# maxnorman569/Variational-Gridded-Gaussian-Processes

Measured on AMD Instinct MI355X. Metric: ELBO-step grid-points/sec (value + 5-component gradient), 1024x1024 RBF grid per GPU, higher is better.
Workload: dtype f64; 1 GPU; 2D Kronecker rbf GP (points basis), 1024x1024 grid (1024x1024 per GPU), m_d=128, Adam fit loop (lr 0.01), eigensolver warm start on; parallelism=single GPU

## Files before the change

include/vggp.h:

```cpp
#ifndef VGGP_H
#define VGGP_H

#include <stdint.h>

#ifdef __cplusplus
extern "C" {
#endif

#define VGGP_VERSION 200

#define VGGP_OK        0
#define VGGP_EINVAL   -1
#define VGGP_ENOTPD   -2
#define VGGP_EHIP     -3
#define VGGP_ENOMEM   -4
#define VGGP_ESTATE   -5
#define VGGP_ENOCONV  -6
#define VGGP_ERCCL    -7

#define VGGP_KIND_MATERN12 0
#define VGGP_KIND_MATERN32 1
#define VGGP_KIND_MATERN52 2
#define VGGP_KIND_RBF      3

// ... 131 lines not shown
                              double* var, vggp_info* info, void* stream);
int vggp_exact_readout_iter(vggp_ctx* ctx, const double* C1, int64_t mv1, const double* C2, int64_t mv2, const double* kd1,
                            const double* kd2, const int64_t* cells, int64_t n_cells, double tol, int max_iter, double* mean, double* var,
                            int flags, vggp_info* info, void* stream);

int vggp_exact_kmv(vggp_ctx* ctx, int kind1, int kind2, double ell1, double ell2, const double* xr1, const double* xr2, int64_t Nr,
                   const double* xc1, const double* xc2, int64_t Nc, const double* V, int64_t nb, double* out0, double* out1, double* out2,
                   void* stream);

int vggp_factor_build(vggp_ctx* ctx, int kind, int basis, const double* x, int64_t n,
                      const double* grid, int64_t m, double ell, int flags,
                      double* A0, double* dA0, double* K0, double* dK0, void* stream);

int vggp_cholesky_inverse(vggp_ctx* ctx, const double* K, int64_t m, double* L, double* Linv,
                          double* jitter_out, void* stream);

int vggp_eigh(vggp_ctx* ctx, const double* G, int64_t m, double* lam, double* Qt,
              int32_t* sweeps_out, int flags, void* stream);

int vggp_gemm(vggp_ctx* ctx, const double* A, int64_t sa_m, int64_t sa_k,
              const double* B, int64_t sb_k, int64_t sb_n,
              double* C, int64_t ldc, int64_t M, int64_t N, int64_t K, void* stream);

int vggp_trsm(vggp_ctx* ctx, const double* L, int64_t m, const double* R, int64_t ncols, double* X, int trans, void* stream);

int vggp_kron_solve(vggp_ctx* ctx, const double* L1, int64_t n1, const double* L2, int64_t n2,
                    const double* Y, double* X, void* stream);

#define VGGP_NSTAGE 20
int         vggp_profile(vggp_ctx* ctx, int enable);
int         vggp_profile_read(vggp_ctx* ctx, double ms_out[VGGP_NSTAGE], int32_t* steps_out, int reset);
const char* vggp_stage_name(int stage);
const char* vggp_project_kernel_name(void);

int vggp_sumsq(vggp_ctx* ctx, const double* y, int64_t n, double* out, void* stream);

#ifdef __cplusplus
}
#endif
#endif
```

variational_gridded_gaussian_processes_amd/_lib.py:

```python
from __future__ import annotations

import ctypes as C
import os

HERE = os.path.dirname(os.path.abspath(__file__))
LIB_PATH = os.path.join(HERE, "libvggp_hip.so")

VGGP_OK, VGGP_EINVAL, VGGP_ENOTPD, VGGP_EHIP, VGGP_ENOMEM, VGGP_ESTATE, VGGP_ENOCONV, VGGP_ERCCL = 0, -1, -2, -3, -4, -5, -6, -7
UNIQUE_ID_BYTES = 128
ALLREDUCE_FN = C.CFUNCTYPE(C.c_int, C.c_void_p, C.POINTER(C.c_double), C.c_int64)
KIND = {"matern12": 0, "matern32": 1, "matern52": 2, "rbf": 3}
NSTAGE = 20
FLAG_B0_F32_KDELTA = 1
FLAG_BLOCK_JACOBI = 2
FLAG_SCATTERED = 4
FLAG_PAIRED_Z = 8
BASIS = {"points": 0, "b0": 1, "one": 2, "vff": 3, "b1": 4}


class VggpError(RuntimeError):
    def __init__(self, code: int, msg: str):
        super().__init__(f"libvggp_hip: {msg} (code {code})")
        self.code = code


class Desc(C.Structure):
    _fields_ = [("kind1", C.c_int32), ("basis1", C.c_int32), ("kind2", C.c_int32), ("basis2", C.c_int32),
                ("n1", C.c_int64), ("n2", C.c_int64), ("m1", C.c_int64), ("m2", C.c_int64),
                ("n_total", C.c_int64),
                ("x1", C.c_void_p), ("x2", C.c_void_p), ("grid1", C.c_void_p), ("grid2", C.c_void_p),
                ("warm_start", C.c_int32), ("flags", C.c_int32)]


class Info(C.Structure):
    _fields_ = [("jitter1", C.c_double), ("jitter2", C.c_double),
                ("sweeps1", C.c_int32), ("sweeps2", C.c_int32),
                ("rounds1", C.c_int32), ("rounds2", C.c_int32),
                ("status", C.c_int32), ("polished", C.c_int32)]

# ... 39 lines not shown
    "vggp_zgrad_scattered": (_I, [_P, _P, _P, _P, _P]),
    "vggp_set_inducing": (_I, [_P, C.c_int, _P, C.c_int64]),
    "vggp_posterior": (_I, [_P, _P, _P, _I64, _P, _P, _P]),
    "vggp_readout": (_I, [_P, _P, _I64, _P, _I64, _P, _P, _P, _P, _I, _P]),
    "vggp_readout_masked": (_I, [_P, _P, _I64, _P, _I64, _P, _P, _P, _P, _I, _P]),
    "vggp_posterior_masked": (_I, [_P, _P, _P, _I64, _P, _P, _P]),
    "vggp_posterior_cov": (_I, [_P, _P, _P, _I64, _P, _P]),
    "vggp_posterior_cov_masked": (_I, [_P, _P, _P, _I64, _P, _P]),
    "vggp_qv_cov_masked": (_I, [_P, _P, _P]),
    "vggp_exact_plan": (_I, [_P, _I, _I, _P, _P, _I64]),
    "vggp_exact_step": (_I, [_P, _P, C.POINTER(_D), C.POINTER(_D), C.POINTER(_D), C.POINTER(Info), _P]),
    "vggp_exact_posterior": (_I, [_P, _P, _P, _I64, _P, _P, _P]),
    "vggp_exact_posterior_cov": (_I, [_P, _P, _P, _I64, _P, _P]),
    "vggp_exact_readout": (_I, [_P, _P, _I64, _P, _I64, _P, _P, _P, _P, _I, _P]),
    "vggp_exact_iter_plan": (_I, [_P, _I, _I, _P, _P, _I64]),
    "vggp_exact_step_iter": (_I, [_P, _P, C.POINTER(_D), _I, _I, _D, _I, C.POINTER(_D), C.POINTER(_D), C.POINTER(Info), _P]),
    "vggp_exact_posterior_iter": (_I, [_P, _P, _P, _I64, _D, _I, _P, _P, C.POINTER(Info), _P]),
    "vggp_exact_readout_iter": (_I, [_P, _P, _I64, _P, _I64, _P, _P, C.POINTER(_I64), _I64, _D, _I, _P, _P, _I, C.POINTER(Info), _P]),
    "vggp_exact_kmv": (_I, [_P, _I, _I, _D, _D, _P, _P, _I64, _P, _P, _I64, _P, _I64, _P, _P, _P, _P]),
    "vggp_factor_build": (_I, [_P, _I, _I, _P, _I64, _P, _I64, _D, _I, _P, _P, _P, _P, _P]),
    "vggp_cholesky_inverse": (_I, [_P, _P, _I64, _P, _P, C.POINTER(_D), _P]),
    "vggp_eigh": (_I, [_P, _P, _I64, _P, _P, C.POINTER(C.c_int32), _I, _P]),
    "vggp_gemm": (_I, [_P, _P, _I64, _I64, _P, _I64, _I64, _P, _I64, _I64, _I64, _I64, _P]),
    "vggp_kron_solve": (_I, [_P, _P, _I64, _P, _I64, _P, _P, _P]),
    "vggp_trsm": (_I, [_P, _P, _I64, _P, _I64, _P, _I, _P]),
    "vggp_sumsq": (_I, [_P, _P, _I64, C.POINTER(_D), _P]),
    "vggp_profile": (_I, [_P, _I]),
    "vggp_profile_read": (_I, [_P, C.POINTER(_D), C.POINTER(C.c_int32), _I]),
    "vggp_stage_name": (C.c_char_p, [_I]),
    "vggp_project_kernel_name": (C.c_char_p, []),
}

_lib = None


def load() -> C.CDLL:
    global _lib
    if _lib is not None:
        return _lib
    if not os.path.exists(LIB_PATH):
        raise ImportError(
            f"{LIB_PATH} not found: build it with `python -m variational_gridded_gaussian_processes_amd.build` "
            "(needs hipcc); there is no CPU fallback")
    lib = C.CDLL(LIB_PATH)
    for name, (res, args) in SYMBOLS.items():
        fn = getattr(lib, name)
# ... 11 lines not shown
```

variational_gridded_gaussian_processes_amd/csrc/api.hip:

```cpp
#include "common.h"

#include <math.h>
#include <stdarg.h>
#include <stdio.h>
#include <stdlib.h>
#include <string.h>
#include <time.h>

#include <algorithm>
#include <vector>

static thread_local char g_err[512] = "";
void vg_set_error(const char* fmt, ...) {
    va_list ap;
    va_start(ap, fmt);
    vsnprintf(g_err, sizeof(g_err), fmt, ap);
    va_end(ap);
}
extern "C" const char* vggp_last_error(void) { return g_err; }
extern "C" int vggp_version(void) { return VGGP_VERSION; }

#include "ctx.h"
#include "factor_elem.h"
#define VG_CHOL_MAXJOBS_HOST 8
// ... 2061 lines not shown
    j.err = counters + 4;
    VG_HIP(vg_eigh_launch(&j, 1, st));
    int hc[8] = {0, 0, 0, 0, 0, 0, 0, 0};
    VG_HIP(hipMemcpyAsync(hc, counters, sizeof(hc), hipMemcpyDeviceToHost, st));
    VG_HIP(hipStreamSynchronize(st));
    if (sweeps_out) *sweeps_out = hc[1] & 0xff;
    if (hc[2] || hc[4]) { vg_set_error("vggp_eigh: no convergence"); return VGGP_ENOCONV; }
    return VGGP_OK;
}

extern "C" int vggp_gemm(vggp_ctx* c, const double* A, int64_t sa_m, int64_t sa_k, const double* B, int64_t sb_k,
                         int64_t sb_n, double* C, int64_t ldc, int64_t M, int64_t N, int64_t K, void* stream) {
    if (!c) { vg_set_error("null context"); return VGGP_EINVAL; }
    VG_REQUIRE(A && B && C && M >= 1 && N >= 1 && K >= 1 && ldc >= N, "vggp_gemm: bad argument");
    VG_REQUIRE(M < (1L << 30) && N < (1L << 30) && K < (1L << 30), "vggp_gemm: dimension too large");
    VG_ENTER_DEVICE(c->device);
    VgGemmBatch g;
    vg_gemm_init(&g);
    vg_gemm_add(&g, A, sa_m, sa_k, B, sb_k, sb_n, C, (int)ldc, (int)M, (int)N, (int)K);
    VG_HIP(vg_gemm_launch(&g, stream ? (hipStream_t)stream : c->own_stream));
    return VGGP_OK;
}

extern "C" int vggp_trsm(vggp_ctx* c, const double* L, int64_t m, const double* R, int64_t ncols, double* X, int trans,
                         void* stream) {
    if (!c) { vg_set_error("null context"); return VGGP_EINVAL; }
    VG_REQUIRE(L && R && X && m >= 1 && m <= 16384 && ncols >= 1, "vggp_trsm: bad argument (1 <= m <= 16384)");
    VG_REQUIRE(m * ncols < (1L << 31) && m * m < (1L << 31), "vggp_trsm: matrix too large");
    VG_ENTER_DEVICE(c->device);
    hipStream_t st = stream ? (hipStream_t)stream : c->own_stream;
    const long nb16 = (m + 15) / 16;
    int rc = vg_ensure_misc(c, (size_t)nb16 * 256 * sizeof(double));
    if (rc) return rc;
    double* Dinv = (double*)c->misc;
    VG_HIP(vg_tri_diaginv_launch(L, m, (int)m, Dinv, st));
    if (X != R) VG_HIP(hipMemcpyAsync(X, R, sizeof(double) * m * ncols, hipMemcpyDeviceToDevice, st));
    return trsm_inplace(L, m, m, Dinv, X, ncols, 1, ncols, trans ? 1 : 0, st);
}

struct VgTriInvSpec { const double* L; long n; const double* Dinv16; double* Xinv; double* tmp; };
static int tri_inverse_batch(const VgTriInvSpec* sp, int nf, hipStream_t st) {
    VgTrsmJob tj[16];
    int nt = 0;
    for (int f = 0; f < nf; ++f)
        for (long r0 = 0; r0 < sp[f].n; r0 += VG_TRSM_BLK) {
            const long rb = std::min<long>(VG_TRSM_BLK, sp[f].n - r0);
// ... 278 lines not shown
```

variational_gridded_gaussian_processes_amd/csrc/common.h:

```cpp
#pragma once
#if defined(__HIP_DEVICE_COMPILE__) && !defined(__gfx950__)
#error "libvggp_hip is written for gfx950 (MI355X) only: kernels rely on its wave64 barrier semantics, MFMA shapes and LDS size"
#endif
#include <hip/hip_runtime.h>
#include <stdint.h>
#include "../../include/vggp.h"

#define VG_WAVE 64

void vg_set_error(const char* fmt, ...);
#define VG_HIP(call)                                                              \
    do {                                                                          \
        hipError_t _e = (call);                                                   \
        if (_e != hipSuccess) {                                                   \
            vg_set_error("%s:%d: %s -> %s", __FILE__, __LINE__, #call,            \
                         hipGetErrorString(_e));                                  \
            return VGGP_EHIP;                                                     \
        }                                                                         \
    } while (0)
#define VG_REQUIRE(cond, ...)                                                     \
    do {                                                                          \
        if (!(cond)) {                                                            \
            vg_set_error(__VA_ARGS__);                                            \
            return VGGP_EINVAL;                                                   \
// ... 42 lines not shown
    double* dot_out;
    int dotw_ld;
    int deep;
    int rev;
};
#define VG_TRI_NONE 0
#define VG_TRI_A_LOWER 1
#define VG_TRI_A_UPPER 2
#define VG_TRI_B_UPPER 3
#define VG_TRI_B_LOWER 4
#define VG_TRI_A_UPPER_B_LOWER 5
struct VgGemmBatch {
    int nprob;
    int total_tiles;
    VgGemmP p[VG_GEMM_MAXP];
};

void vg_gemm_init(VgGemmBatch* b);
int vg_gemm_add(VgGemmBatch* b, const double* A, long sa_m, long sa_k, const double* B, long sb_k,
                long sb_n, double* C, int ldc, int M, int N, int K, int ksplit = 1, long c_slab = 0,
                int b_nslab = 1, long b_slab = 0, double alpha = 1.0, int accum = 0);
#define VG_GEMM_TAG_GRAM_PROJECT 1
#define VG_GEMM_TAG_WIDE 2
void vg_gemm_xcd_group(VgGemmBatch* b, int prob);
hipError_t vg_gemm_launch(const VgGemmBatch* b, hipStream_t st, int tag = 0);
const char* vg_last_project_kernel();

#define VG_RED_MAXSEG 8
struct VgRedSeg { const double* in; double* out; long n; long slab; int nslab; int block_start; };
struct VgRedBatch { int nseg; int total_blocks; VgRedSeg s[VG_RED_MAXSEG]; };
void vg_red_init(VgRedBatch* b);
void vg_red_add(VgRedBatch* b, const double* in, double* out, long n, long slab, int nslab);
hipError_t vg_red_launch(const VgRedBatch* b, hipStream_t st);

struct VgFactorJob {
    const double* x;
    const double* grid;
    double* A0;
    double* dA0;
    double* K0;
    double* dK0;
    int n, m, kind, basis;
    int theta_idx;
    double ell_imm;
    int flags;
};
// ... 183 lines not shown
```

variational_gridded_gaussian_processes_amd/csrc/gemm.hip:

```cpp
#include "gemm_body.h"

#include <cstdint>
#include <cstdio>
#include <cstdlib>

__global__ __launch_bounds__(256) void vg_gemm_kernel(const VgGemmBatch b) {
    __shared__ double lds[2 * VgTile<64, 16>::TILE];
    vg_gemm_body<64, 16>(b, lds, blockIdx.x);
}
__global__ __launch_bounds__(256) void vg_gemm_gram_project_kernel(const VgGemmBatch b) {
    __shared__ double lds[2 * VgTile<64, 16>::TILE];
    vg_gemm_body<64, 16>(b, lds, blockIdx.x);
}
__global__ __launch_bounds__(512) void vg_gemm_gram_project_wide_kernel(const VgGemmBatch b) {
    __shared__ double lds[2 * VgTile<64, 16>::TILE];
    vg_gemm_body<64, 16, 512>(b, lds, blockIdx.x);
}
typedef double vg_d2 __attribute__((ext_vector_type(2)));
__global__ __launch_bounds__(512) void vg_gemm_project_deep_kernel(const VgGemmBatch b) {
    constexpr int T = 64, NT = 512, BK = 32;
    constexpr int RS = BK + 2;
    constexpr int KS = T + 16;
    constexpr int NA = T * BK / (2 * NT);
    __shared__ __attribute__((aligned(16))) double lds[T * RS + BK * KS];
// ... 184 lines not shown
        for (int i = 0; i < out->nprob; ++i) {
            const VgGemmP& p = out->p[i];
            fprintf(stderr, "[deep] NOT deep: prob %d/%d M %d N %d K %d ksplit %d kchunk %d sa (%ld,%ld) sb (%ld,%ld) aslab %d bslab %d tri %d accum %d tiles %d deep %d\n",
                    i, out->nprob, p.M, p.N, p.K, p.ksplit, p.kchunk, p.sa_m, p.sa_k, p.sb_k, p.sb_n, p.a_nslab, p.b_nslab, p.tri, p.accum,
                    p.tiles_m * p.tiles_n * p.ksplit, p.deep);
        }
    return 4 * deep_tiles >= 3L * out->total_tiles;
}
__global__ __launch_bounds__(512) void vg_gemm_deep_kernel(const VgGemmBatch b) {
    constexpr int DT = 32 * 80 > 64 * 34 ? 32 * 80 : 64 * 34;
    __shared__ __attribute__((aligned(16))) double lds[2 * DT];
    const int bid = blockIdx.x;
    int pi = 0;
    for (int i = 1; i < b.nprob; ++i)
        if (bid >= b.p[i].tile_start) pi = i;
    if (b.p[pi].deep) vg_gemm_deep_body(b.p[pi], lds, bid - b.p[pi].tile_start);
    else vg_gemm_body<64, 16, 512>(b, lds, bid);
}
__global__ __launch_bounds__(512) void vg_gemm_wide_kernel(const VgGemmBatch b) {
    __shared__ double lds[2 * VgTile<64, 16>::TILE];
    vg_gemm_body<64, 16, 512>(b, lds, blockIdx.x);
}
__global__ __launch_bounds__(256) void vg_gemm_small_kernel(const VgGemmBatch b) {
    __shared__ double lds[2 * VgTile<32, 32>::TILE];
    vg_gemm_body<32, 32>(b, lds, blockIdx.x);
}

void vg_gemm_init(VgGemmBatch* b) {
    b->nprob = 0;
    b->total_tiles = 0;
}

int vg_gemm_add(VgGemmBatch* b, const double* A, long sa_m, long sa_k, const double* B, long sb_k,
                long sb_n, double* C, int ldc, int M, int N, int K, int ksplit, long c_slab,
                int b_nslab, long b_slab, double alpha, int accum) {
    if (b->nprob >= VG_GEMM_MAXP) return -1;
    VgGemmP& p = b->p[b->nprob];
    p.A = A; p.B = B; p.C = C;
    p.sa_m = sa_m; p.sa_k = sa_k; p.sb_k = sb_k; p.sb_n = sb_n;
    p.M = M; p.N = N; p.K = K; p.ldc = ldc;
    p.alpha = alpha; p.accum = accum;
    if (ksplit < 1) ksplit = 1;
    int ktiles = (K + VG_BK - 1) / VG_BK;
    if (ktiles < 1) ktiles = 1;
    if (ksplit > ktiles) ksplit = ktiles;
    int per = (ktiles + ksplit - 1) / ksplit;
// ... 11 lines not shown
    p.dotw = nullptr; p.dot_out = nullptr; p.dotw_ld = 0; p.deep = 0;
    p.tiles_m = (M + VG_BM - 1) / VG_BM;
    p.tiles_n = (N + VG_BN - 1) / VG_BN;
    p.tile_start = b->total_tiles;
    b->total_tiles += p.tiles_m * p.tiles_n * ksplit;
    return b->nprob++;
}

void vg_gemm_xcd_group(VgGemmBatch* b, int prob) {
    static const bool off = getenv("VGGP_NO_XCD_GROUP") != nullptr;
    VgGemmP& p = b->p[prob];
    const bool ok = !off && p.tile_start == 0 && (p.ksplit == 1 || p.ksplit == 2 || p.ksplit == 4 || p.ksplit == 8) &&
                    (p.tiles_n % (8 / p.ksplit)) == 0;
    p.xcd_group = ok ? 1 : 0;
}

static bool vg_deep_batch(const VgGemmBatch* b, VgGemmBatch* out);

static const char* g_last_project_kernel = "";
const char* vg_last_project_kernel() { return g_last_project_kernel; }

hipError_t vg_gemm_launch(const VgGemmBatch* b, hipStream_t st, int tag) {
    if (b->nprob == 0 || b->total_tiles == 0) return hipSuccess;
    bool small = b->total_tiles < 128;
    for (int i = 0; i < b->nprob; ++i) small = small && b->p[i].ksplit == 1 && b->p[i].K <= 512;
    if (small) {
        VgGemmBatch s = *b;
        s.total_tiles = 0;
        for (int i = 0; i < s.nprob; ++i) {
            VgGemmP& p = s.p[i];
            p.tiles_m = (p.M + 31) / 32;
            p.tiles_n = (p.N + 31) / 32;
            p.kchunk = ((p.K + 31) / 32) * 32;
            p.xcd_group = 0;
            p.tile_start = s.total_tiles;
            s.total_tiles += p.tiles_m * p.tiles_n;
        }
        hipLaunchKernelGGL(vg_gemm_small_kernel, dim3(s.total_tiles), dim3(256), 0, st, s);
        return hipGetLastError();
    }
    static const bool wide = getenv("VGGP_GEMM_NARROW") == nullptr;
    VgGemmBatch deepb;
    if (tag == VG_GEMM_TAG_GRAM_PROJECT && wide && vg_project_deep_ok(b)) {
        g_last_project_kernel = "vg_gemm_project_deep_kernel";
        hipLaunchKernelGGL(vg_gemm_project_deep_kernel, dim3(b->total_tiles), dim3(512), 0, st, *b);
    } else if (tag == VG_GEMM_TAG_GRAM_PROJECT && wide && b->total_tiles <= 320) {
        g_last_project_kernel = "vg_gemm_gram_project_wide_kernel";
        hipLaunchKernelGGL(vg_gemm_gram_project_wide_kernel, dim3(b->total_tiles), dim3(512), 0, st, *b);
    } else if (tag == VG_GEMM_TAG_GRAM_PROJECT) {
        g_last_project_kernel = "vg_gemm_gram_project_kernel";
        hipLaunchKernelGGL(vg_gemm_gram_project_kernel, dim3(b->total_tiles), dim3(256), 0, st, *b);
    }
    else if (vg_deep_batch(b, &deepb)) {
        hipLaunchKernelGGL(vg_gemm_deep_kernel, dim3(deepb.total_tiles), dim3(512), 0, st, deepb);
    }
    else if (tag == VG_GEMM_TAG_WIDE && wide && b->total_tiles <= 320)
        hipLaunchKernelGGL(vg_gemm_wide_kernel, dim3(b->total_tiles), dim3(512), 0, st, *b);
    else
        hipLaunchKernelGGL(vg_gemm_kernel, dim3(b->total_tiles), dim3(256), 0, st, *b);
    return hipGetLastError();
}
// ... 38 lines not shown
```

variational_gridded_gaussian_processes_amd/csrc/gemm_body.h:

```cpp
#pragma once
#include "common.h"

typedef double vg_d4 __attribute__((ext_vector_type(4)));

template <int T, int BK>
struct VgTile {
    static constexpr int RPAD = BK == 16 ? 1 : 4;
    static constexpr int RS = BK + RPAD;
    static constexpr int KS = T + 16;
    static constexpr int TILE = (BK * KS > T * RS) ? BK * KS : T * RS;
    static constexpr int MB = T / 32;
};

template <int T, int BK, int NT = 256>
__device__ __forceinline__ void vg_gemm_body(const VgGemmBatch& b, double* lds, const int bid) {
    using C_ = VgTile<T, BK>;
    constexpr int NR = T * BK / NT;
    constexpr int WC = NT / 128;
    constexpr int MB = T / 32;
    constexpr int NB = T / (16 * WC);
    double* As = lds;
    double* Bs = lds + C_::TILE;

    int pi = 0;
    for (int i = 1; i < b.nprob; ++i)
        if (bid >= b.p[i].tile_start) pi = i;
    const VgGemmP& p = b.p[pi];

    int t = bid - p.tile_start;
    const int tiles = p.tiles_m * p.tiles_n;
    int ks, tm, tn;
    if (p.xcd_group) {
        const int nx = 8 / p.ksplit;
        const int xcd = t & 7, j = t >> 3;
        ks = xcd / nx;
        const int gi = j / p.tiles_m;
        tm = j - gi * p.tiles_m;
// ... 90 lines not shown
            Bs[b_k[r] * b_sk + b_j[r] * b_sj] = rb[r];
        }
        __syncthreads();
        if (knext < k_end) load_tile(knext, ra, rb);
#pragma unroll
        for (int kk = 0; kk < BK; kk += 4) {
            double av[MB], bv[NB];
#pragma unroll
            for (int mb = 0; mb < MB; ++mb)
                av[mb] = As[(wr * WT + mb * 16 + fi) * a_si + (kk + fk) * a_sk];
#pragma unroll
            for (int nb = 0; nb < NB; ++nb)
                bv[nb] = Bs[(kk + fk) * b_sk + (wc * WTC + nb * 16 + fi) * b_sj];
#pragma unroll
            for (int mb = 0; mb < MB; ++mb)
#pragma unroll
                for (int nb = 0; nb < NB; ++nb)
                    acc[mb][nb] = __builtin_amdgcn_mfma_f64_16x16x4f64(av[mb], bv[nb], acc[mb][nb], 0, 0, 0);
        }
        __syncthreads();
    };
    const bool fast = row0 + T <= M && col0 + T <= N && k_begin < k_end && ((k_end - k_begin) % BK) == 0 &&
                      ((nslab == 1 && anslab == 1) || p.K <= 512);
    if (fast) {
        const double* pa[NR];
        const double* pb[NR];
        int la[NR], lb[NR];
#pragma unroll
        for (int r = 0; r < NR; ++r) {
            pa[r] = A + (long)(row0 + a_i[r]) * sa_m + (long)(k_begin + a_k[r]) * sa_k;
            pb[r] = B + (long)(k_begin + b_k[r]) * sb_k + (long)(col0 + b_j[r]) * sb_n;
            la[r] = a_i[r] * a_si + a_k[r] * a_sk;
            lb[r] = b_k[r] * b_sk + b_j[r] * b_sj;
        }
        const long da = (long)BK * sa_k, db = (long)BK * sb_k;
        const int nk = (k_end - k_begin) / BK;
        auto ld = [&](double (&ra)[NR], double (&rb)[NR]) {
#pragma unroll
            for (int r = 0; r < NR; ++r) { ra[r] = *pa[r]; rb[r] = *pb[r]; }
            for (int sl = 1; sl < nslab; sl += 3) {
                const long o0 = (long)sl * bslab, o1 = sl + 1 < nslab ? o0 + bslab : o0, o2 = sl + 2 < nslab ? o0 + 2 * bslab : o0;
                const double w1 = sl + 1 < nslab ? 1.0 : 0.0, w2 = sl + 2 < nslab ? 1.0 : 0.0;
#pragma unroll
                for (int r = 0; r < NR; ++r) rb[r] += (pb[r][o0] + w1 * pb[r][o1]) + w2 * pb[r][o2];
            }
            for (int sl = 1; sl < anslab; sl += 3) {
                const long o0 = (long)sl * aslab, o1 = sl + 1 < anslab ? o0 + aslab : o0, o2 = sl + 2 < anslab ? o0 + 2 * aslab : o0;
// ... 77 lines not shown
```

variational_gridded_gaussian_processes_amd/csrc/thin.hip:

```cpp
#include "common.h"

typedef double vt_d4 __attribute__((ext_vector_type(4)));

#define VT_MAXR 32
#define VT_NBUF 15
#define VT_NBIG 11
#define VT_NSMALL 14
#ifdef VGGP_DIAG
#define VT_STAMP(i) do { if (threadIdx.x == 0 && tt.stamps) { unsigned long long t_; asm volatile("s_memrealtime %0\n\ts_waitcnt lgkmcnt(0)" : "=s"(t_) :: "memory"); tt.stamps[i] = t_; } } while (0)
#else
#define VT_STAMP(i)
#endif

struct VtTask { int c, a, sa_i, sa_k, b; };

__device__ __forceinline__ void vt_mm(double* base, int sz, const VtTask* tk, int ntask, int mp, int ld, int kk) {
    const int lane = threadIdx.x & 63, wave = threadIdx.x >> 6, nw = blockDim.x >> 6, nb = mp >> 4;
    const int fi = lane & 15, fk = lane >> 4;
    for (int t = wave; t < ntask * nb * nb; t += nw) {
        const int task = t / (nb * nb), blk = t - task * nb * nb, bi = blk / nb, bj = blk - bi * nb;
        const VtTask T = tk[task];
        const double* a = base + (long)T.a * sz + (bi * 16 + fi) * T.sa_i + fk * T.sa_k;
        const double* b = base + (long)T.b * sz + fk * ld + bj * 16 + fi;
        double* C = base + (long)T.c * sz;
// ... 27 lines not shown
        for (int q = 0; q < NV; ++q) t[q] = __shfl_xor(v[q], off);
#pragma unroll
        for (int q = 0; q < NV; ++q) v[q] += t[q];
    }
}

enum { B_W1 = 0, B_W1T, B_W2, B_W2T, B_E1, B_F1, B_E2, B_F2, B_P0, B_P1, B_P2, B_T0, B_T1, B_T2, B_T3 };

__global__ __launch_bounds__(1024) void vg_thin_tail_kernel(const VgThinTail tt) {
    extern __shared__ __attribute__((aligned(16))) double vt_dyn[];
    __shared__ double red[16 * VT_NBIG], tot[VT_NBIG + VT_NSMALL];
    __shared__ double dg[4][256];
    __shared__ double l1s[VT_MAXR], l2s[VT_MAXR], rs1[VT_MAXR], rl1[VT_MAXR], rs2[VT_MAXR], rl2[VT_MAXR];
    __shared__ VtTask tk[18];
    __shared__ double stage[16];
    __shared__ double jit_s[2], pf_s, seq_s;
    __shared__ int rc_s[2][4], st_s[2][2];
    const int r1 = tt.r1, r2 = tt.r2, tid = threadIdx.x, nthr = blockDim.x;
    const int rmax = r1 > r2 ? r1 : r2, mp = (rmax + 15) & ~15, ld = mp + 2, sz = mp * ld;
    double* base = vt_dyn;
    const double s1 = tt.theta[2], s2 = tt.theta[3], v = tt.theta[4];

    VT_STAMP(0);
    for (int e = tid; e < sz; e += nthr) {
        const int i = e / ld, j = e - i * ld;
        const bool in1 = i < r1 && j < r1, in2 = i < r2 && j < r2, in12 = i < r1 && j < r2;
        const double w1 = in1 ? tt.W1[i * r1 + j] : 0.0, w2 = in2 ? tt.W2[i * r2 + j] : 0.0;
        const double am1 = in1 ? tt.AM1[i * r1 + j] : 0.0, ah1 = in1 ? tt.AH1[i * r1 + j] : 0.0;
        const double am2 = in2 ? tt.AM2[i * r2 + j] : 0.0, ah2 = in2 ? tt.AH2[i * r2 + j] : 0.0;
        double c0 = 0.0, c1 = 0.0, c2 = 0.0;
        if (in12)
            for (int sl = 0; sl < tt.ac_nslab; ++sl) {
                const double* ac = tt.AC + sl * tt.ac_slab + i * r2 + j;
                c0 += ac[0]; c1 += ac[(long)r1 * r2]; c2 += ac[2L * r1 * r2];
            }
        base[B_W1 * sz + e] = w1; base[B_W2 * sz + e] = w2;
        if (j < mp) { base[B_W1T * sz + j * ld + i] = w1; base[B_W2T * sz + j * ld + i] = w2; }
        base[B_E1 * sz + e] = am1; base[B_F1 * sz + e] = ah1; base[B_E2 * sz + e] = am2; base[B_F2 * sz + e] = ah2;
        base[B_P0 * sz + e] = c0; base[B_P1 * sz + e] = c1; base[B_P2 * sz + e] = c2;
    }
    if (tid < VT_MAXR) {
        l1s[tid] = tid < r1 ? s1 * tt.lam1[tid] : 0.0;
        l2s[tid] = tid < r2 ? s2 * tt.lam2[tid] : 0.0;
    }
    if (tid >= 64 && tid < 72) { const int k = (tid - 64) >> 2, q = (tid - 64) & 3; rc_s[k][q] = tt.rcounters[k] ? tt.rcounters[k][q] : 0; }
    if (tid >= 72 && tid < 76) { const int k = (tid - 72) >> 1, q = (tid - 72) & 1; st_s[k][q] = tt.status[k] ? tt.status[k][q] : 0; }
    if (tid >= 76 && tid < 78) jit_s[tid - 76] = tt.jit[tid - 76] ? *tt.jit[tid - 76] : 0.0;
    if (tid == 78) pf_s = tt.peer_fail ? *tt.peer_fail : 0.0;
    if (tid == 79) seq_s = tt.theta[5];
    if (tid >= 128 && tid < 384) {
        const int i = tid - 128;
        dg[0][i] = i < tt.m1 ? tt.G1[(long)i * tt.m1 + i] : 0.0; dg[1][i] = i < tt.m1 ? tt.H1[(long)i * tt.m1 + i] : 0.0;
        dg[2][i] = i < tt.m2 ? tt.G2[(long)i * tt.m2 + i] : 0.0; dg[3][i] = i < tt.m2 ? tt.H2[(long)i * tt.m2 + i] : 0.0;
    }
    if (tid == 0) {
        tk[0] = VtTask{B_T0, B_E1, ld, 1, B_W1T}; tk[1] = VtTask{B_T1, B_F1, ld, 1, B_W1T};
        tk[2] = VtTask{B_T2, B_E2, ld, 1, B_W2T}; tk[3] = VtTask{B_T3, B_F2, ld, 1, B_W2T};
        tk[4] = VtTask{B_E1, B_W1, ld, 1, B_T0}; tk[5] = VtTask{B_F1, B_W1, ld, 1, B_T1};
        tk[6] = VtTask{B_E2, B_W2, ld, 1, B_T2}; tk[7] = VtTask{B_F2, B_W2, ld, 1, B_T3};
        tk[8] = VtTask{B_T0, B_P0, ld, 1, B_W2T}; tk[9] = VtTask{B_T1, B_P1, ld, 1, B_W2T}; tk[10] = VtTask{B_T2, B_P2, ld, 1, B_W2T};
        tk[11] = VtTask{B_P0, B_W1, ld, 1, B_T0}; tk[12] = VtTask{B_P1, B_W1, ld, 1, B_T1}; tk[13] = VtTask{B_P2, B_W1, ld, 1, B_T2};
        tk[14] = VtTask{B_W1, B_T0, ld, 1, B_T1}; tk[15] = VtTask{B_W1T, B_T2, ld, 1, B_T1};
        tk[16] = VtTask{B_W2, B_T0, 1, ld, B_T0}; tk[17] = VtTask{B_P0, B_T3, 1, ld, B_T0};
    }
    VT_STAMP(1);
    __syncthreads();
    VT_STAMP(2);

    const int kk = (rmax + 7) & ~7;
    vt_mm(base, sz, tk, 4, mp, ld, kk);
    vt_mm(base, sz, tk + 4, 4, mp, ld, kk);
    VT_STAMP(3);
    vt_mm(base, sz, tk + 8, 3, mp, ld, kk);
    vt_mm(base, sz, tk + 11, 3, mp, ld, kk);
    VT_STAMP(4);

// ... 221 lines not shown
```

variational_gridded_gaussian_processes_amd/engine.py:

```python
from __future__ import annotations

import ctypes as C
from typing import Optional, Sequence, Tuple

import numpy as np
import torch

from . import _lib
from ._lib import BASIS, KIND, Desc, Info, check


def _ptr(t: Optional[torch.Tensor]) -> Optional[int]:
    if t is None:
        return None
    if not (t.is_cuda and t.dtype == torch.float64 and t.is_contiguous()):
        raise TypeError("engine tensors must be contiguous float64 on the GPU")
    return t.data_ptr()


def _stream(device=None) -> int:
    return torch.cuda.current_stream(device).cuda_stream


def _dvec(x) -> np.ndarray:
# ... 576 lines not shown
        return L, Li, jit.value

    def eigh(self, G: torch.Tensor, block: bool = False):
        m = G.shape[0]
        lam = torch.empty(m, dtype=torch.float64, device=self.device)
        Qt = torch.empty_like(G)
        sw = C.c_int32()
        check(self.lib.vggp_eigh(self._h, _ptr(G), m, _ptr(lam), _ptr(Qt), C.byref(sw),
                                 _lib.FLAG_BLOCK_JACOBI if block else 0, _stream(self.device)))
        return lam, Qt, sw.value

    def gemm(self, A: torch.Tensor, B: torch.Tensor) -> torch.Tensor:
        M, K = A.shape
        K2, N = B.shape
        assert K == K2
        Cm = torch.empty(M, N, dtype=torch.float64, device=self.device)
        for t in (A, B):
            if not (t.is_cuda and t.dtype == torch.float64):
                raise TypeError("gemm operands must be float64 GPU tensors")
        check(self.lib.vggp_gemm(self._h, A.data_ptr(), A.stride(0), A.stride(1), B.data_ptr(), B.stride(0),
                                 B.stride(1), Cm.data_ptr(), N, M, N, K, _stream(self.device)))
        return Cm

    def kron_solve(self, L1: torch.Tensor, L2: torch.Tensor, Y: torch.Tensor) -> torch.Tensor:
        n1, n2 = Y.shape
        X = torch.empty_like(Y)
        check(self.lib.vggp_kron_solve(self._h, _ptr(L1), n1, _ptr(L2), n2, _ptr(Y), _ptr(X), _stream(self.device)))
        return X

    def trsm(self, L: torch.Tensor, R: torch.Tensor, trans: bool = False) -> torch.Tensor:
        m, ncols = R.shape
        X = torch.empty_like(R)
        check(self.lib.vggp_trsm(self._h, _ptr(L), m, _ptr(R), ncols, _ptr(X), 1 if trans else 0, _stream(self.device)))
        return X

    def profile(self, enable: bool = True) -> None:
        check(self.lib.vggp_profile(self._h, 1 if enable else 0))

    def profile_read(self, reset: bool = True):
        ms = (C.c_double * _lib.NSTAGE)()
        steps = C.c_int32()
        check(self.lib.vggp_profile_read(self._h, ms, C.byref(steps), 1 if reset else 0))
        names = [self.lib.vggp_stage_name(i).decode() for i in range(_lib.NSTAGE)]
        return dict(zip(names, list(ms))), steps.value

    def project_kernel_name(self) -> str:
# ... 7 lines not shown
```

Before: 5.409 billion grid-points/s.

## Batch slab-sum loads in small GEMM and restructure thin-kernel prologue loads

Adds a batched slab-summing k-tile path to the small GEMM kernel. It issues all slab loads for a k-tile together in registers and double-buffers them, instead of reducing slabs serially, and keeps the old serial kernel behind a flag or environment variable. It also rewrites the thin kernel's prologue so each thread issues its global loads up front, with different waves fetching the scalar metadata and diagonals in parallel, to hide load latency. The cost is much higher register pressure in the small GEMM, and summation order changes for slab counts above 8.

```diff
diff --git a/include/vggp.h b/include/vggp.h
--- a/include/vggp.h
+++ b/include/vggp.h
@@ -177,6 +177,11 @@
               const double* B, int64_t sb_k, int64_t sb_n,
               double* C, int64_t ldc, int64_t M, int64_t N, int64_t K, void* stream);
 
+#define VGGP_GEMM_SLAB_SERIAL 1
+int vggp_gemm_slabs(vggp_ctx* ctx, const double* A, int64_t sa_m, int64_t sa_k, int64_t a_nslab, int64_t a_slab,
+                    const double* B, int64_t sb_k, int64_t sb_n, int64_t b_nslab, int64_t b_slab,
+                    double* C, int64_t ldc, int64_t M, int64_t N, int64_t K, int flags, void* stream);
+
 int vggp_trsm(vggp_ctx* ctx, const double* L, int64_t m, const double* R, int64_t ncols, double* X, int trans, void* stream);
 
 int vggp_kron_solve(vggp_ctx* ctx, const double* L1, int64_t n1, const double* L2, int64_t n2,
diff --git a/variational_gridded_gaussian_processes_amd/_lib.py b/variational_gridded_gaussian_processes_amd/_lib.py
--- a/variational_gridded_gaussian_processes_amd/_lib.py
+++ b/variational_gridded_gaussian_processes_amd/_lib.py
@@ -15,6 +15,7 @@
 FLAG_BLOCK_JACOBI = 2
 FLAG_SCATTERED = 4
 FLAG_PAIRED_Z = 8
+GEMM_SLAB_SERIAL = 1
 BASIS = {"points": 0, "b0": 1, "one": 2, "vff": 3, "b1": 4}
 
 
@@ -100,6 +101,7 @@
     "vggp_cholesky_inverse": (_I, [_P, _P, _I64, _P, _P, C.POINTER(_D), _P]),
     "vggp_eigh": (_I, [_P, _P, _I64, _P, _P, C.POINTER(C.c_int32), _I, _P]),
     "vggp_gemm": (_I, [_P, _P, _I64, _I64, _P, _I64, _I64, _P, _I64, _I64, _I64, _I64, _P]),
+    "vggp_gemm_slabs": (_I, [_P, _P, _I64, _I64, _I64, _I64, _P, _I64, _I64, _I64, _I64, _P, _I64, _I64, _I64, _I64, _I, _P]),
     "vggp_kron_solve": (_I, [_P, _P, _I64, _P, _I64, _P, _P, _P]),
     "vggp_trsm": (_I, [_P, _P, _I64, _P, _I64, _P, _I, _P]),
     "vggp_sumsq": (_I, [_P, _P, _I64, C.POINTER(_D), _P]),
diff --git a/variational_gridded_gaussian_processes_amd/csrc/api.hip b/variational_gridded_gaussian_processes_amd/csrc/api.hip
--- a/variational_gridded_gaussian_processes_amd/csrc/api.hip
+++ b/variational_gridded_gaussian_processes_amd/csrc/api.hip
@@ -2107,6 +2107,22 @@
     return VGGP_OK;
 }
 
+extern "C" int vggp_gemm_slabs(vggp_ctx* c, const double* A, int64_t sa_m, int64_t sa_k, int64_t a_nslab, int64_t a_slab,
+                               const double* B, int64_t sb_k, int64_t sb_n, int64_t b_nslab, int64_t b_slab, double* C, int64_t ldc,
+                               int64_t M, int64_t N, int64_t K, int flags, void* stream) {
+    if (!c) { vg_set_error("null context"); return VGGP_EINVAL; }
+    VG_REQUIRE(A && B && C && M >= 1 && N >= 1 && K >= 1 && ldc >= N, "vggp_gemm_slabs: bad argument");
+    VG_REQUIRE(M < (1L << 30) && N < (1L << 30) && K < (1L << 30), "vggp_gemm_slabs: dimension too large");
+    VG_REQUIRE(a_nslab >= 1 && a_nslab <= 64 && b_nslab >= 1 && b_nslab <= 64, "vggp_gemm_slabs: 1 <= nslab <= 64");
+    VG_ENTER_DEVICE(c->device);
+    VgGemmBatch g;
+    vg_gemm_init(&g);
+    const int i = vg_gemm_add(&g, A, sa_m, sa_k, B, sb_k, sb_n, C, (int)ldc, (int)M, (int)N, (int)K, 1, 0, (int)b_nslab, b_slab);
+    g.p[i].a_nslab = (int)a_nslab; g.p[i].a_slab = a_slab;
+    VG_HIP(vg_gemm_launch(&g, stream ? (hipStream_t)stream : c->own_stream, (flags & VGGP_GEMM_SLAB_SERIAL) ? VG_GEMM_TAG_SLAB_SERIAL : 0));
+    return VGGP_OK;
+}
+
 extern "C" int vggp_trsm(vggp_ctx* c, const double* L, int64_t m, const double* R, int64_t ncols, double* X, int trans,
                          void* stream) {
     if (!c) { vg_set_error("null context"); return VGGP_EINVAL; }
diff --git a/variational_gridded_gaussian_processes_amd/csrc/common.h b/variational_gridded_gaussian_processes_amd/csrc/common.h
--- a/variational_gridded_gaussian_processes_amd/csrc/common.h
+++ b/variational_gridded_gaussian_processes_amd/csrc/common.h
@@ -88,6 +88,7 @@
                 int b_nslab = 1, long b_slab = 0, double alpha = 1.0, int accum = 0);
 #define VG_GEMM_TAG_GRAM_PROJECT 1
 #define VG_GEMM_TAG_WIDE 2
+#define VG_GEMM_TAG_SLAB_SERIAL 3
 void vg_gemm_xcd_group(VgGemmBatch* b, int prob);
 hipError_t vg_gemm_launch(const VgGemmBatch* b, hipStream_t st, int tag = 0);
 const char* vg_last_project_kernel();
diff --git a/variational_gridded_gaussian_processes_amd/csrc/gemm.hip b/variational_gridded_gaussian_processes_amd/csrc/gemm.hip
--- a/variational_gridded_gaussian_processes_amd/csrc/gemm.hip
+++ b/variational_gridded_gaussian_processes_amd/csrc/gemm.hip
@@ -230,6 +230,10 @@
     vg_gemm_body<64, 16, 512>(b, lds, blockIdx.x);
 }
 __global__ __launch_bounds__(256) void vg_gemm_small_kernel(const VgGemmBatch b) {
+    __shared__ double lds[2 * VgTile<32, 32>::TILE];
+    vg_gemm_body<32, 32, 256, true>(b, lds, blockIdx.x);
+}
+__global__ __launch_bounds__(256) void vg_gemm_small_serial_kernel(const VgGemmBatch b) {
     __shared__ double lds[2 * VgTile<32, 32>::TILE];
     vg_gemm_body<32, 32>(b, lds, blockIdx.x);
 }
@@ -287,6 +291,8 @@
 
 hipError_t vg_gemm_launch(const VgGemmBatch* b, hipStream_t st, int tag) {
     if (b->nprob == 0 || b->total_tiles == 0) return hipSuccess;
+    static const bool serial = getenv("VGGP_SLAB_SERIAL") != nullptr;
+    const bool legacy = serial || tag == VG_GEMM_TAG_SLAB_SERIAL;
     bool small = b->total_tiles < 128;
     for (int i = 0; i < b->nprob; ++i) small = small && b->p[i].ksplit == 1 && b->p[i].K <= 512;
     if (small) {
@@ -301,7 +307,8 @@
             p.tile_start = s.total_tiles;
             s.total_tiles += p.tiles_m * p.tiles_n;
         }
-        hipLaunchKernelGGL(vg_gemm_small_kernel, dim3(s.total_tiles), dim3(256), 0, st, s);
+        if (legacy) hipLaunchKernelGGL(vg_gemm_small_serial_kernel, dim3(s.total_tiles), dim3(256), 0, st, s);
+        else hipLaunchKernelGGL(vg_gemm_small_kernel, dim3(s.total_tiles), dim3(256), 0, st, s);
         return hipGetLastError();
     }
     static const bool wide = getenv("VGGP_GEMM_NARROW") == nullptr;
diff --git a/variational_gridded_gaussian_processes_amd/csrc/gemm_body.h b/variational_gridded_gaussian_processes_amd/csrc/gemm_body.h
--- a/variational_gridded_gaussian_processes_amd/csrc/gemm_body.h
+++ b/variational_gridded_gaussian_processes_amd/csrc/gemm_body.h
@@ -1,5 +1,7 @@
 #pragma once
 #include "common.h"
+
+#include <type_traits>
 
 typedef double vg_d4 __attribute__((ext_vector_type(4)));
 
@@ -12,7 +14,135 @@
     static constexpr int MB = T / 32;
 };
 
-template <int T, int BK, int NT = 256>
+template <int T, int BK, int NT>
+__device__ __forceinline__ void vg_gemm_slab_ktiles(const VgGemmP& p, double* lds, const int row0, const int col0, const int k_begin,
+                                                    const int k_end, vg_d4 (&acc)[T / 32][T / (16 * (NT / 128))]) {
+    using C_ = VgTile<T, BK>;
+    constexpr int NR = T * BK / NT, WC = NT / 128, MB = T / 32, NB = T / (16 * WC), WT = T / 2, WTC = T / WC;
+    constexpr int SL = 8, TL = 8;
+    const int tid = threadIdx.x, lane = tid & 63, wave = tid >> 6;
+    const int wr = wave / WC, wc = wave % WC, fi = lane & 15, fk = lane >> 4;
+    const bool a_kc = p.sa_k == 1, b_nc = p.sb_n == 1;
+    const int a_si = a_kc ? C_::RS : 1, a_sk = a_kc ? 1 : C_::KS;
+    const int b_sj = b_nc ? 1 : C_::RS, b_sk = b_nc ? C_::KS : 1;
+    const bool xb = p.b_nslab > 1;
+    const double* __restrict__ X = xb ? p.B : p.A;
+    const double* __restrict__ Y = xb ? p.A : p.B;
+    const long xsk = xb ? p.sb_k : p.sa_k, ysk = xb ? p.sa_k : p.sb_k;
+    const int n = xb ? p.b_nslab : p.a_nslab;
+    const long xslab = xb ? p.b_slab : p.a_slab;
+    const int nsum = n > SL ? 1 : n;
+    long xo[NR], yo[NR];
+    int xk[NR], yk[NR], lx[NR], ly[NR];
+    bool xin[NR], yin[NR];
+#pragma unroll
+    for (int r = 0; r < NR; ++r) {
+        int ai, ak, bk, bj;
+        if (a_kc) { ak = tid % BK; ai = tid / BK + (NT / BK) * r; }
+        else      { ai = tid % T; ak = tid / T + (NT / T) * r; }
+        if (b_nc) { bj = tid % T; bk = tid / T + (NT / T) * r; }
+        else      { bk = tid % BK; bj = tid / BK + (NT / BK) * r; }
+        const long ao = (long)(row0 + ai) * p.sa_m + (long)ak * p.sa_k, bo = (long)bk * p.sb_k + (long)(col0 + bj) * p.sb_n;
+        const int la = ai * a_si + ak * a_sk, lb = C_::TILE + bk * b_sk + bj * b_sj;
+        const bool ain = row0 + ai < p.M, bin = col0 + bj < p.N;
+        xo[r] = xb ? bo : ao; yo[r] = xb ? ao : bo;
+        xk[r] = xb ? bk : ak; yk[r] = xb ? ak : bk;
+        lx[r] = xb ? lb : la; ly[r] = xb ? la : lb;
+        xin[r] = xb ? bin : ain; yin[r] = xb ? ain : bin;
+    }
+    long so[SL], to[TL];
+#pragma unroll
+    for (int s = 0; s < SL; ++s) so[s] = s < n ? s * xslab : 0;
+#pragma unroll
+    for (int u = 0; u < TL; ++u) to[u] = SL + u < n ? (SL + u) * xslab : 0;
+
+    auto ld = [&](const int k0, double (&ry)[NR], double (&rx)[SL][NR]) {
+        const double* q[NR];
+#pragma unroll
+        for (int r = 0; r < NR; ++r) {
+            const bool okx = xin[r] && k0 + xk[r] < k_end, oky = yin[r] && k0 + yk[r] < k_end;
+            q[r] = X + (okx ? xo[r] + k0 * xsk : 0);
+            ry[r] = Y[oky ? yo[r] + k0 * ysk : 0];
+#pragma unroll
+            for (int s = 0; s < SL; ++s) rx[s][r] = q[r][so[s]];
+        }
+        if (n > SL) {
+            double t[TL][NR];
+#pragma unroll
+            for (int u = 0; u < TL; ++u)
+#pragma unroll
+                for (int r = 0; r < NR; ++r) t[u][r] = q[r][to[u]];
+#pragma unroll
+            for (int r = 0; r < NR; ++r) {
+                double v = rx[0][r];
+                v += (rx[1][r] + rx[2][r]) + rx[3][r];
+                v += (rx[4][r] + rx[5][r]) + rx[6][r];
+                v += (rx[7][r] + t[0][r]) + (n > 9 ? t[1][r] : 0.0);
+                if (n > 10) v += (t[2][r] + (n > 11 ? t[3][r] : 0.0)) + (n > 12 ? t[4][r] : 0.0);
+                if (n > 13) v += (t[5][r] + (n > 14 ? t[6][r] : 0.0)) + (n > 15 ? t[7][r] : 0.0);
+                rx[0][r] = v;
+            }
+        }
+    };
+    auto kt = [&](const int k0, double (&ry)[NR], double (&rx)[SL][NR], auto more) {
+#pragma unroll
+        for (int r = 0; r < NR; ++r) {
+            double v = rx[0][r];
+#pragma unroll
+            for (int g = 1; g < SL; g += 3) {
+                double grp = rx[g][r];
+                if (g + 1 < SL) grp += g + 1 < nsum ? rx[g + 1][r] : 0.0;
+                if (g + 2 < SL) grp += g + 2 < nsum ? rx[g + 2][r] : 0.0;
+                v = g < nsum ? v + grp : v;
+            }
+            lds[lx[r]] = (xin[r] && k0 + xk[r] < k_end) ? v : 0.0;
+            lds[ly[r]] = (yin[r] && k0 + yk[r] < k_end) ? ry[r] : 0.0;
+        }
+        __syncthreads();
+        if constexpr (decltype(more)::value) ld(k0 + 2 * BK, ry, rx);
+        const double* As = lds;
+        const double* Bs = lds + C_::TILE;
+#pragma unroll
+        for (int kk = 0; kk < BK; kk += 4) {
+            double av[MB], bv[NB];
+#pragma unroll
+            for (int mb = 0; mb < MB; ++mb) av[mb] = As[(wr * WT + mb * 16 + fi) * a_si + (kk + fk) * a_sk];
+#pragma unroll
+            for (int nb = 0; nb < NB; ++nb) bv[nb] = Bs[(kk + fk) * b_sk + (wc * WTC + nb * 16 + fi) * b_sj];
+#pragma unroll
+            for (int mb = 0; mb < MB; ++mb)
+#pragma unroll
+                for (int nb = 0; nb < NB; ++nb)
+                    acc[mb][nb] = __builtin_amdgcn_mfma_f64_16x16x4f64(av[mb], bv[nb], acc[mb][nb], 0, 0, 0);
+        }
+        __syncthreads();
+    };
+    using Yes = std::true_type;
+    using No = std::false_type;
+
+    double y0[NR], x0[SL][NR], y1[NR], x1[SL][NR];
+    const int nk = k_begin < k_end ? (k_end - k_begin + BK - 1) / BK : 0;
+    int k0 = k_begin;
+    if (nk & 1) {
+        ld(k0, y1, x1);
+        ld(k0 + BK, y0, x0);
+        kt(k0, y1, x1, Yes());
+        k0 += BK;
+    } else {
+        ld(k0, y0, x0);
+        ld(k0 + BK, y1, x1);
+    }
+    for (; k0 + 2 * BK < k_end; k0 += 2 * BK) {
+        kt(k0, y0, x0, Yes());
+        kt(k0 + BK, y1, x1, Yes());
+    }
+    if (k0 < k_end) {
+        kt(k0, y0, x0, No());
+        kt(k0 + BK, y1, x1, No());
+    }
+}
+
+template <int T, int BK, int NT = 256, bool BATCH = false>
 __device__ __forceinline__ void vg_gemm_body(const VgGemmBatch& b, double* lds, const int bid) {
     using C_ = VgTile<T, BK>;
     constexpr int NR = T * BK / NT;
@@ -149,7 +279,10 @@
     };
     const bool fast = row0 + T <= M && col0 + T <= N && k_begin < k_end && ((k_end - k_begin) % BK) == 0 &&
                       ((nslab == 1 && anslab == 1) || p.K <= 512);
-    if (fast) {
+    const bool batched = BATCH && (nslab > 1) != (anslab > 1) && nslab <= 16 && anslab <= 16;
+    if (batched) {
+        if constexpr (BATCH) vg_gemm_slab_ktiles<T, BK, NT>(p, lds, row0, col0, k_begin, k_end, acc);
+    } else if (fast) {
         const double* pa[NR];
         const double* pb[NR];
         int la[NR], lb[NR];
diff --git a/variational_gridded_gaussian_processes_amd/csrc/thin.hip b/variational_gridded_gaussian_processes_amd/csrc/thin.hip
--- a/variational_gridded_gaussian_processes_amd/csrc/thin.hip
+++ b/variational_gridded_gaussian_processes_amd/csrc/thin.hip
@@ -73,36 +73,64 @@
     const double s1 = tt.theta[2], s2 = tt.theta[3], v = tt.theta[4];
 
     VT_STAMP(0);
-    for (int e = tid; e < sz; e += nthr) {
-        const int i = e / ld, j = e - i * ld;
-        const bool in1 = i < r1 && j < r1, in2 = i < r2 && j < r2, in12 = i < r1 && j < r2;
-        const double w1 = in1 ? tt.W1[i * r1 + j] : 0.0, w2 = in2 ? tt.W2[i * r2 + j] : 0.0;
-        const double am1 = in1 ? tt.AM1[i * r1 + j] : 0.0, ah1 = in1 ? tt.AH1[i * r1 + j] : 0.0;
-        const double am2 = in2 ? tt.AM2[i * r2 + j] : 0.0, ah2 = in2 ? tt.AH2[i * r2 + j] : 0.0;
-        double c0 = 0.0, c1 = 0.0, c2 = 0.0;
-        if (in12)
-            for (int sl = 0; sl < tt.ac_nslab; ++sl) {
-                const double* ac = tt.AC + sl * tt.ac_slab + i * r2 + j;
-                c0 += ac[0]; c1 += ac[(long)r1 * r2]; c2 += ac[2L * r1 * r2];
-            }
+    const int wave = __builtin_amdgcn_readfirstlane(tid >> 6), lane = tid & 63;
+    const int i = tid / mp, j = tid - i * mp;
+    const bool el = tid < mp * mp;
+    const bool in1 = el && i < r1 && j < r1, in2 = el && i < r2 && j < r2, in12 = el && i < r1 && j < r2;
+    const int o1 = in1 ? i * r1 + j : 0, o2 = in2 ? i * r2 + j : 0;
+    const double* ac = tt.AC + (in12 ? i * r2 + j : 0);
+    const double w1g = tt.W1[o1], w2g = tt.W2[o2], am1g = tt.AM1[o1], ah1g = tt.AH1[o1], am2g = tt.AM2[o2], ah2g = tt.AH2[o2];
+    double c0 = 0.0 + ac[0], c1 = 0.0 + ac[(long)r1 * r2], c2 = 0.0 + ac[2L * r1 * r2];
+    double lm1 = 0.0, lm2 = 0.0, dword = 0.0, d0 = 0.0, d1 = 0.0, d2 = 0.0, d3 = 0.0;
+    int iword = 0;
+    if (wave == 0) {
+        lm1 = tt.lam1[lane < r1 ? lane : 0];
+        lm2 = tt.lam2[lane < r2 ? lane : 0];
+    } else if (wave == 1) {
+        const int* pk = (lane & 4) ? tt.rcounters[1] : tt.rcounters[0];
+        const int* pl = pk ? pk : reinterpret_cast<const int*>(tt.theta);
+        iword = pl[lane & 3];
+        iword = pk ? iword : 0;
+    } else if (wave == 2) {
+        const int* pk = (lane & 2) ? tt.status[1] : tt.status[0];
+        const int* pl = pk ? pk : reinterpret_cast<const int*>(tt.theta);
+        iword = pl[lane & 1];
+        iword = pk ? iword : 0;
+    } else if (wave == 3) {
+        const double* pk = lane == 0 ? tt.jit[0] : lane == 1 ? tt.jit[1] : lane == 2 ? tt.peer_fail : tt.theta + 5;
+        dword = *(pk ? pk : tt.theta);
+        dword = pk ? dword : 0.0;
+    } else if (wave < 8) {
+        const int q = tid - 256;
+        const long q1 = q < tt.m1 ? (long)q * tt.m1 + q : 0, q2 = q < tt.m2 ? (long)q * tt.m2 + q : 0;
+        d0 = tt.G1[q1]; d1 = tt.H1[q1]; d2 = tt.G2[q2]; d3 = tt.H2[q2];
+    }
+    for (int sl = 1; sl < tt.ac_nslab; ++sl) {
+        const double* as = ac + sl * tt.ac_slab;
+        c0 += as[0]; c1 += as[(long)r1 * r2]; c2 += as[2L * r1 * r2];
+    }
+    if (el) {
+        const int e = i * ld + j, et = j * ld + i;
+        const double w1 = in1 ? w1g : 0.0, w2 = in2 ? w2g : 0.0;
         base[B_W1 * sz + e] = w1; base[B_W2 * sz + e] = w2;
-        if (j < mp) { base[B_W1T * sz + j * ld + i] = w1; base[B_W2T * sz + j * ld + i] = w2; }
-        base[B_E1 * sz + e] = am1; base[B_F1 * sz + e] = ah1; base[B_E2 * sz + e] = am2; base[B_F2 * sz + e] = ah2;
-        base[B_P0 * sz + e] = c0; base[B_P1 * sz + e] = c1; base[B_P2 * sz + e] = c2;
+        base[B_W1T * sz + et] = w1; base[B_W2T * sz + et] = w2;
+        base[B_E1 * sz + e] = in1 ? am1g : 0.0; base[B_F1 * sz + e] = in1 ? ah1g : 0.0;
+        base[B_E2 * sz + e] = in2 ? am2g : 0.0; base[B_F2 * sz + e] = in2 ? ah2g : 0.0;
+        base[B_P0 * sz + e] = in12 ? c0 : 0.0; base[B_P1 * sz + e] = in12 ? c1 : 0.0; base[B_P2 * sz + e] = in12 ? c2 : 0.0;
     }
     if (tid < VT_MAXR) {
-        l1s[tid] = tid < r1 ? s1 * tt.lam1[tid] : 0.0;
-        l2s[tid] = tid < r2 ? s2 * tt.lam2[tid] : 0.0;
-    }
-    if (tid >= 64 && tid < 72) { const int k = (tid - 64) >> 2, q = (tid - 64) & 3; rc_s[k][q] = tt.rcounters[k] ? tt.rcounters[k][q] : 0; }
-    if (tid >= 72 && tid < 76) { const int k = (tid - 72) >> 1, q = (tid - 72) & 1; st_s[k][q] = tt.status[k] ? tt.status[k][q] : 0; }
-    if (tid >= 76 && tid < 78) jit_s[tid - 76] = tt.jit[tid - 76] ? *tt.jit[tid - 76] : 0.0;
-    if (tid == 78) pf_s = tt.peer_fail ? *tt.peer_fail : 0.0;
-    if (tid == 79) seq_s = tt.theta[5];
-    if (tid >= 128 && tid < 384) {
-        const int i = tid - 128;
-        dg[0][i] = i < tt.m1 ? tt.G1[(long)i * tt.m1 + i] : 0.0; dg[1][i] = i < tt.m1 ? tt.H1[(long)i * tt.m1 + i] : 0.0;
-        dg[2][i] = i < tt.m2 ? tt.G2[(long)i * tt.m2 + i] : 0.0; dg[3][i] = i < tt.m2 ? tt.H2[(long)i * tt.m2 + i] : 0.0;
+        l1s[tid] = tid < r1 ? s1 * lm1 : 0.0;
+        l2s[tid] = tid < r2 ? s2 * lm2 : 0.0;
+    }
+    if (wave == 1 && lane < 8) rc_s[lane >> 2][lane & 3] = iword;
+    if (wave == 2 && lane < 4) st_s[lane >> 1][lane & 1] = iword;
+    if (wave == 3 && lane < 2) jit_s[lane] = dword;
+    if (wave == 3 && lane == 2) pf_s = dword;
+    if (wave == 3 && lane == 3) seq_s = dword;
+    if (wave >= 4 && wave < 8) {
+        const int q = tid - 256;
+        dg[0][q] = q < tt.m1 ? d0 : 0.0; dg[1][q] = q < tt.m1 ? d1 : 0.0;
+        dg[2][q] = q < tt.m2 ? d2 : 0.0; dg[3][q] = q < tt.m2 ? d3 : 0.0;
     }
     if (tid == 0) {
         tk[0] = VtTask{B_T0, B_E1, ld, 1, B_W1T}; tk[1] = VtTask{B_T1, B_F1, ld, 1, B_W1T};
diff --git a/variational_gridded_gaussian_processes_amd/engine.py b/variational_gridded_gaussian_processes_amd/engine.py
--- a/variational_gridded_gaussian_processes_amd/engine.py
+++ b/variational_gridded_gaussian_processes_amd/engine.py
@@ -622,6 +622,20 @@
                                  B.stride(1), Cm.data_ptr(), N, M, N, K, _stream(self.device)))
         return Cm
 
+    def gemm_slabs(self, A: torch.Tensor, B: torch.Tensor, serial: bool = False) -> torch.Tensor:
+        for t in (A, B):
+            if not (t.is_cuda and t.dtype == torch.float64 and t.dim() in (2, 3)):
+                raise TypeError("gemm_slabs operands must be 2-D or 3-D float64 GPU tensors")
+        A3 = A if A.dim() == 3 else A.unsqueeze(0)
+        B3 = B if B.dim() == 3 else B.unsqueeze(0)
+        (na, M, K), (nb, K2, N) = A3.shape, B3.shape
+        assert K == K2
+        Cm = torch.empty(M, N, dtype=torch.float64, device=self.device)
+        check(self.lib.vggp_gemm_slabs(self._h, A3.data_ptr(), A3.stride(1), A3.stride(2), na, A3.stride(0) if na > 1 else 0,
+                                       B3.data_ptr(), B3.stride(1), B3.stride(2), nb, B3.stride(0) if nb > 1 else 0,
+                                       Cm.data_ptr(), N, M, N, K, _lib.GEMM_SLAB_SERIAL if serial else 0, _stream(self.device)))
+        return Cm
+
     def kron_solve(self, L1: torch.Tensor, L2: torch.Tensor, Y: torch.Tensor) -> torch.Tensor:
         n1, n2 = Y.shape
         X = torch.empty_like(Y)
```

After: 5.466 billion grid-points/s, median of 4. No clear change (+1.1%).
